# kevaday/alphazero-general

Measured on AMD Instinct MI355X. Metric: mcts_node_expansions_per_sec, higher is better.
Workload: dtype f32 tree / f16 net; 1 GPU; connect4 self-play, 2048 games/GPU x 100 sims/move, fp16 ResNet 128ch x 8, random-init, noise+temp on; games_per_gpu=2048, sims_per_move=100, hipgraph_rounds=True, stream_pipelines=1, fused_search_launch=True, mfma_tower=True, ranks=1

## Files before the change

alphazero_general_amd/csrc/azg_engine.hip:

```cpp
#include <hip/hip_runtime.h>
#include <hip/hip_ext.h>
#include <cstdio>
#include <cstdlib>
#include <cstring>
#include <map>
#include <mutex>
#include <string>
#include <vector>
#include "azg_kernels.h"
#include "azg_rules.h"
#include "azg_conv.h"
#include "azg_tiles.h"

using namespace azg;

static thread_local std::string g_err;
static int fail(int code, const std::string &msg) { g_err = msg; return code; }
#define HIPCHK(x) do { hipError_t _e = (x); if (_e != hipSuccess) return fail(AZG_E_HIP, std::string(#x) + ": " + hipGetErrorString(_e)); } while (0)

struct EvPair { hipEvent_t a, b; bool ext; };

static thread_local EvPair *g_kev = nullptr;
#define AZG_LAUNCH(kernel, grid, block, lds, stream, ...) do { \
    if (g_kev) { hipExtLaunchKernelGGL(kernel, grid, block, lds, stream, g_kev->a, g_kev->b, 0, __VA_ARGS__); g_kev = nullptr; } \
// ... 56 lines not shown
    e->allocs.push_back(q);
    *p = (T *)q;
    return AZG_OK;
}
#define DALLOC(ptr, count) do { int _r = dalloc(e, &(ptr), (size_t)(count)); if (_r != AZG_OK) return _r; } while (0)

#define AZG_GAME_CASE(G_, ...) case G_::ID: { using G = G_; __VA_ARGS__; } break;
#define GAME_SWITCH(e, ...) \
    switch ((e)->cfg.game) { AZG_GAMES(AZG_GAME_CASE, __VA_ARGS__) default: return fail(AZG_E_UNSUPPORTED, "game has no device rules"); }
#define AZG_SPARSE_CASE(G_, ...) case G_::ID: if constexpr (G_::SPARSE_HEADS) { using G = G_; __VA_ARGS__; } \
    else return fail(AZG_E_UNSUPPORTED, std::string("no sparse heads for ") + G_::NAME + " (use the dense heads)"); break;
#define SPARSE_GAME_SWITCH(e, ...) \
    switch ((e)->cfg.game) { AZG_GAMES(AZG_SPARSE_CASE, __VA_ARGS__) default: return fail(AZG_E_UNSUPPORTED, "game has no device rules"); }
#define OBS_SWITCH(obs_dtype, obs, CALL) \
    if ((obs_dtype) == 0) { using OBS = float; constexpr bool NHWC8 = false; OBS *const o = (OBS *)(obs); CALL; } \
    else if ((obs_dtype) == 1) { using OBS = _Float16; constexpr bool NHWC8 = false; OBS *const o = (OBS *)(obs); CALL; } \
    else { using OBS = _Float16; constexpr bool NHWC8 = true; OBS *const o = (OBS *)(obs); CALL; }

static void prof_begin(azg_engine *e, hipStream_t s, int fam, EvPair &p) {
    if (!e->profile) return;
    if (!e->pool.empty()) { p = e->pool.back(); e->pool.pop_back(); }
    else { (void)hipEventCreate(&p.a); (void)hipEventCreate(&p.b); }
    p.ext = fam != 2;
    if (p.ext) g_kev = &p; else (void)hipEventRecord(p.a, s);
}
static void prof_end(azg_engine *e, hipStream_t s, int fam, EvPair &p) {
    if (!e->profile) return;
    if (!p.ext) (void)hipEventRecord(p.b, s);
    g_kev = nullptr;
    e->ev[fam].push_back(p);
    e->launches[fam]++;
}
static void prof_drain(azg_engine *e) {
    for (int f = 0; f < 3; f++) {
        for (auto &p : e->ev[f]) {
            (void)hipEventSynchronize(p.b);
            float t = 0; (void)hipEventElapsedTime(&t, p.a, p.b);
            e->ms[f] += t;
            e->pool.push_back(p);
        }
        e->ev[f].clear();
    }
}

extern "C" int azg_engine_create(const azg_config *cfg, azg_engine **out) {
    if (!cfg || !out) return fail(AZG_E_INVALID_ARG, "null argument");
    if (cfg->abi_version != AZG_ABI_VERSION) return fail(AZG_E_INVALID_ARG, "ABI version mismatch");
    if (cfg->game < 0 || cfg->game >= k_num_games) return fail(AZG_E_UNSUPPORTED, "game has no device rules");
    if (cfg->num_slots <= 0) return fail(AZG_E_INVALID_ARG, "num_slots must be > 0");
    int ndev = 0;
    if (hipGetDeviceCount(&ndev) != hipSuccess || ndev == 0)
        return fail(AZG_E_HIP, "no HIP device: libazg_hip has no CPU fallback");
    HIPCHK(hipSetDevice(cfg->device));
    azg_engine *e = new azg_engine();
    e->cfg = *cfg; e->gi = k_info[cfg->game];
    const azg_game_info &gi = e->gi;
    View &v = e->v;
    memset(&v, 0, sizeof(v));
    v.B = cfg->num_slots; v.arena = cfg->arena ? 1 : 0; v.T = v.arena ? gi.num_players : 1;
    const int sims = cfg->sims_per_move > 0 ? cfg->sims_per_move : 100;
    const long long per_move = (long long)sims * gi.max_children;
    const long long cap = cfg->nodes_per_tree > 0 ? cfg->nodes_per_tree : (long long)(gi.max_turns < 16 ? gi.max_turns : 16) * per_move + 64;
    if (cap >= (1 << 28)) { delete e; return fail(AZG_E_INVALID_ARG, "nodes_per_tree must be < 2^28"); }
    v.cap = (int)cap;
    v.compact_reserve = (int)(per_move < cap / 2 ? per_move : cap / 2);
    v.maxd = gi.max_turns + 2; v.max_hist = gi.max_turns + 1;
    v.ex_cap = cfg->example_capacity; v.res_cap = cfg->result_capacity > 0 ? cfg->result_capacity : 4 * v.B + 1024;
    v.add_noise = (cfg->add_root_noise && !v.arena) ? 1 : 0; v.add_temp = (cfg->add_root_temp && !v.arena) ? 1 : 0;
    v.symmetric = cfg->symmetric_samples; v.reset_thr = cfg->mcts_reset_threshold; v.games_cap = cfg->games_per_iteration;
    v.cpuct = cfg->cpuct; v.fpu_reduction = cfg->fpu_reduction; v.noise_frac = cfg->root_noise_frac;
    v.root_temp = cfg->root_policy_temp; v.arena_temp = cfg->arena_temp;
    v.seed = cfg->tape_seed; v.slot_base = cfg->slot_base;
    const size_t trees = (size_t)v.B * v.T;
    const int A = gi.action_size, NV = gi.num_players + 1, O = gi.obs_c * gi.obs_h * gi.obs_w;
    DALLOC(v.nodes, trees * 2 * (size_t)v.cap);
    DALLOC(v.hdr, trees);
    DALLOC(v.path, trees * (size_t)v.maxd);
    DALLOC(v.states, v.B); DALLOC(v.leaf_states, v.B);
    DALLOC(v.tape_ctr, v.B); DALLOC(v.next_reset, v.B); DALLOC(v.hist_len, v.B);
    const bool hist = !v.arena && v.ex_cap > 0;
    DALLOC(v.hist_state, hist ? (size_t)v.B * v.max_hist : 1);
    DALLOC(v.hist_pi, hist ? (size_t)v.B * v.max_hist * A : 1);
    if (!hist) v.max_hist = 0;
    DALLOC(v.last_action, v.B); DALLOC(v.fin_flag, v.B); DALLOC(v.fin_ridx, v.B); DALLOC(v.fin_counted, v.B); DALLOC(v.fin_soff, v.B);
    DALLOC(v.slot_sims, v.B); DALLOC(v.slot_exp, v.B);
    DALLOC(v.gcount, 8);
    DALLOC(v.ex_obs, (size_t)v.ex_cap * O); DALLOC(v.ex_pi, (size_t)v.ex_cap * A); DALLOC(v.ex_z, (size_t)v.ex_cap * NV);
    DALLOC(v.res_ws, (size_t)v.res_cap * NV); DALLOC(v.res_turns, v.res_cap); DALLOC(v.res_slot, v.res_cap);
    std::vector<float> tt;
    if (cfg->temp_table && cfg->temp_table_len > 0) tt.assign(cfg->temp_table, cfg->temp_table + cfg->temp_table_len);
    else tt.assign(1, cfg->start_temp);
    float *d_tt; DALLOC(d_tt, tt.size());
    HIPCHK(hipMemcpy(d_tt, tt.data(), tt.size() * sizeof(float), hipMemcpyHostToDevice));
    v.temp_table = d_tt; v.temp_len = (int)tt.size();
    DALLOC(e->d_p2i, 8); DALLOC(e->d_ok, 4);
#ifdef AZG_TREE_TIMING
    DALLOC(v.dbg, (size_t)v.B * 16);
#endif
    *out = e;
    int r = azg_engine_reset(e, nullptr);
    if (r != AZG_OK) { azg_engine_destroy(e); *out = nullptr; return r; }
    HIPCHK(hipDeviceSynchronize());
    return AZG_OK;
}

extern "C" int azg_engine_destroy(azg_engine *e) {
    if (!e) return AZG_OK;
    (void)hipDeviceSynchronize();
    prof_drain(e);
    for (auto &p : e->pool) { (void)hipEventDestroy(p.a); (void)hipEventDestroy(p.b); }
    for (void *p : e->allocs) (void)hipFree(p);
    if (e->d_perm) (void)hipFree(e->d_perm);
    if (e->d_utape) (void)hipFree(e->d_utape);
    if (e->d_noff) (void)hipFree(e->d_noff);
    if (e->d_npool) (void)hipFree(e->d_npool);
    delete e;
    return AZG_OK;
}

extern "C" int azg_engine_reset(azg_engine *e, void *stream) {
    if (!e) return fail(AZG_E_INVALID_ARG, "null engine");
    hipStream_t s = (hipStream_t)stream;
    GAME_SWITCH(e, hipLaunchKernelGGL((k_reset<G>), dim3(e->v.B), dim3(64), 0, s, e->v, 0, e->v.B, 1));
    HIPCHK(hipMemsetAsync(e->v.tape_ctr, 0, sizeof(uint64_t) * e->v.B, s));
    HIPCHK(hipMemsetAsync(e->v.gcount, 0, sizeof(int32_t) * 8, s));
    HIPCHK(hipMemsetAsync(e->v.slot_sims, 0, sizeof(int64_t) * e->v.B, s));
    HIPCHK(hipMemsetAsync(e->v.slot_exp, 0, sizeof(int64_t) * e->v.B, s));
    HIPCHK(hipGetLastError());
    return AZG_OK;
}

static int check_range(azg_engine *e, int first, int count) {
    if (!e) return fail(AZG_E_INVALID_ARG, "null engine");
    if (first < 0 || count < 0 || first + count > e->v.B) return fail(AZG_E_INVALID_ARG, "slot range out of bounds");
    return AZG_OK;
}

extern "C" int azg_set_states(azg_engine *e, void *stream, int first, int count, const azg_state *host, int reset_trees) {
    int r = check_range(e, first, count); if (r) return r;
    hipStream_t s = (hipStream_t)stream;
    HIPCHK(hipMemcpyAsync(e->v.states + first, host, sizeof(azg_state) * count, hipMemcpyHostToDevice, s));
    if (reset_trees) { GAME_SWITCH(e, hipLaunchKernelGGL((k_reset<G>), dim3(count), dim3(64), 0, s, e->v, first, count, 0)); }
    HIPCHK(hipStreamSynchronize(s));
    return AZG_OK;
}
extern "C" int azg_get_states(azg_engine *e, void *stream, int first, int count, azg_state *host) {
    int r = check_range(e, first, count); if (r) return r;
    hipStream_t s = (hipStream_t)stream;
    HIPCHK(hipMemcpyAsync(host, e->v.states + first, sizeof(azg_state) * count, hipMemcpyDeviceToHost, s));
    HIPCHK(hipStreamSynchronize(s));
    return AZG_OK;
}
extern "C" int azg_get_leaf_states(azg_engine *e, void *stream, int first, int count, azg_state *host) {
    int r = check_range(e, first, count); if (r) return r;
    hipStream_t s = (hipStream_t)stream;
    HIPCHK(hipMemcpyAsync(host, e->v.leaf_states + first, sizeof(azg_state) * count, hipMemcpyDeviceToHost, s));
    HIPCHK(hipStreamSynchronize(s));
    return AZG_OK;
}
extern "C" int azg_set_tape_counters(azg_engine *e, void *stream, int first, int count, const uint64_t *host) {
    int r = check_range(e, first, count); if (r) return r;
    hipStream_t s = (hipStream_t)stream;
    HIPCHK(hipMemcpyAsync(e->v.tape_ctr + first, host, sizeof(uint64_t) * count, hipMemcpyHostToDevice, s));
    HIPCHK(hipStreamSynchronize(s));
    return AZG_OK;
}
extern "C" int azg_get_tape_counters(azg_engine *e, void *stream, int first, int count, uint64_t *host) {
// ... 54 lines not shown
    GAME_SWITCH(e, {
        RawValueRow<G> vrow;
        for (int j = 0; j < G::P + 1; j++) vrow.v[j] = value_host[j];
        hipLaunchKernelGGL((k_search_raw<G>), dim3(e->v.B), dim3(64), 0, s, e->v, policy_fill, vrow, sims);
    });
    HIPCHK(hipGetLastError());
    return AZG_OK;
}

extern "C" int azg_backup_select(azg_engine *e, void *stream, const float *policy, const float *value, const int32_t *row_of_slot, int flags,
                                 void *obs, int obs_dtype) {
    if (!e || !policy || !value) return fail(AZG_E_INVALID_ARG, "null argument");
    if (obs_dtype < 0 || obs_dtype > 2) return fail(AZG_E_INVALID_ARG, "obs_dtype must be 0 (f32), 1 (f16) or 2 (f16 NHWC8)");
    hipStream_t s = (hipStream_t)stream;
    View v = e->v;
    if (flags >= 0) { v.add_noise = (flags & AZG_FLAG_NOISE) ? 1 : 0; v.add_temp = (flags & AZG_FLAG_TEMP) ? 1 : 0; }
    EvPair p; prof_begin(e, s, 1, p);
    const int A = e->gi.action_size;
    OBS_SWITCH(obs_dtype, obs, GAME_SWITCH(e, AZG_LAUNCH((k_backup_select2<G, OBS, NHWC8, IN_PROBS>), dim3(v.B), dim3(128), 0, s, v, policy, value, A, o, row_of_slot, 1, HeadRows{})));
    prof_end(e, s, 1, p);
    HIPCHK(hipGetLastError());
    return AZG_OK;
}

extern "C" int azg_backup_select_logits(azg_engine *e, void *stream, const float *logits, int logits_stride, const int32_t *row_of_slot,
                                        int flags, void *obs, int obs_dtype, int do_select) {
    if (!e || !logits) return fail(AZG_E_INVALID_ARG, "null argument");
    if (obs_dtype < 0 || obs_dtype > 2) return fail(AZG_E_INVALID_ARG, "obs_dtype must be 0 (f32), 1 (f16) or 2 (f16 NHWC8)");
    if (logits_stride < e->gi.action_size + e->gi.num_players + 1 || e->gi.action_size > 1024)
        return fail(AZG_E_INVALID_ARG, "logits_stride must hold A + P + 1 logits (A <= 1024)");
    hipStream_t s = (hipStream_t)stream;
    View v = e->v;
    if (flags >= 0) { v.add_noise = (flags & AZG_FLAG_NOISE) ? 1 : 0; v.add_temp = (flags & AZG_FLAG_TEMP) ? 1 : 0; }
    EvPair p; prof_begin(e, s, 1, p);
    const float *nov = nullptr;
    OBS_SWITCH(obs_dtype, obs, GAME_SWITCH(e, AZG_LAUNCH((k_backup_select2<G, OBS, NHWC8, IN_LOGITS>), dim3(v.B), dim3(128), 0, s, v, logits, nov, logits_stride, o, row_of_slot, do_select, HeadRows{})));
    prof_end(e, s, 1, p);
    HIPCHK(hipGetLastError());
    return AZG_OK;
}

extern "C" int azg_backup_select_features(azg_engine *e, void *stream, const void *feat, int feat_k, const void *head_rows, const float *head_b,
                                          const int32_t *row_of_slot, int flags, void *obs, int obs_dtype, int do_select) {
    if (!e || !feat || !head_rows || !head_b) return fail(AZG_E_INVALID_ARG, "null argument");
    if (obs_dtype < 0 || obs_dtype > 2) return fail(AZG_E_INVALID_ARG, "obs_dtype must be 0 (f32), 1 (f16) or 2 (f16 NHWC8)");
    if (e->gi.action_size > 1024) return fail(AZG_E_INVALID_ARG, "A <= 1024");
    hipStream_t s = (hipStream_t)stream;
    View v = e->v;
    if (flags >= 0) { v.add_noise = (flags & AZG_FLAG_NOISE) ? 1 : 0; v.add_temp = (flags & AZG_FLAG_TEMP) ? 1 : 0; }
    const HeadRows hd{(const _Float16 *)head_rows, head_b, feat_k};
    int want = 0;
    SPARSE_GAME_SWITCH(e, want = head_fk<G>());
    if (feat_k != want) return fail(AZG_E_INVALID_ARG, "feat_k must be cells x 16 rounded up to a multiple of 32 for this game");
    EvPair p; prof_begin(e, s, 1, p);
    const float *nov = nullptr, *f = (const float *)feat;
    OBS_SWITCH(obs_dtype, obs, SPARSE_GAME_SWITCH(e, AZG_LAUNCH((k_backup_select2<G, OBS, NHWC8, IN_FEATURES>), dim3(v.B), dim3(128), 0, s, v, f, nov, 0, o, row_of_slot, do_select, hd)));
    prof_end(e, s, 1, p);
    HIPCHK(hipGetLastError());
    return AZG_OK;
}

extern "C" int azg_leaf_heads_sparse_f16(azg_engine *e, void *stream, const void *feat, int feat_k, const void *head_rows, const float *head_b,
                                         const int32_t *row_of_slot, float *logits, int logits_stride) {
    if (!e || !feat || !head_rows || !head_b || !logits) return fail(AZG_E_INVALID_ARG, "null argument");
    if (logits_stride < e->gi.action_size + e->gi.num_players + 1 || e->gi.action_size > 1024)
        return fail(AZG_E_INVALID_ARG, "logits_stride must hold A + P + 1 logits (A <= 1024)");
    int want = 0;
    SPARSE_GAME_SWITCH(e, want = head_fk<G>());
    if (feat_k != want) return fail(AZG_E_INVALID_ARG, "feat_k must be cells x 16 rounded up to a multiple of 32 for this game");
    const HeadRows hd{(const _Float16 *)head_rows, head_b, feat_k};
    SPARSE_GAME_SWITCH(e, hipLaunchKernelGGL((k_leaf_heads_sparse<G>), dim3(e->v.B), dim3(64), 0, (hipStream_t)stream, e->v, (const _Float16 *)feat, hd,
                                      row_of_slot, logits, logits_stride));
    HIPCHK(hipGetLastError());
    return AZG_OK;
}

extern "C" int azg_advance(azg_engine *e, void *stream, int record_history) {
    if (!e) return fail(AZG_E_INVALID_ARG, "null engine");
    hipStream_t s = (hipStream_t)stream;
    EvPair p; prof_begin(e, s, 2, p);
    GAME_SWITCH(e, {
        hipLaunchKernelGGL((k_play<G>), dim3(e->v.B), dim3(64), 0, s, e->v, record_history);
        hipLaunchKernelGGL((k_finalize<G>), dim3(1), dim3(64), 0, s, e->v, (const int32_t *)nullptr);
        hipLaunchKernelGGL((k_emit_samples<G>), dim3(e->v.B, G::NSYM), dim3(64), 0, s, e->v);
        hipLaunchKernelGGL((k_emit<G>), dim3(e->v.B), dim3(64), 0, s, e->v);
        hipLaunchKernelGGL((k_compact<G>), dim3(e->v.B * e->v.T), dim3(64), 0, s, e->v, 0, 0);
    });
    prof_end(e, s, 2, p);
    HIPCHK(hipGetLastError());
    return AZG_OK;
}

extern "C" int azg_advance_begin(azg_engine *e, void *stream, int record_history, int32_t *fin_host) {
    if (!e || !fin_host) return fail(AZG_E_INVALID_ARG, "null argument");
    hipStream_t s = (hipStream_t)stream;
    GAME_SWITCH(e, hipLaunchKernelGGL((k_play<G>), dim3(e->v.B), dim3(64), 0, s, e->v, record_history));
    HIPCHK(hipGetLastError());
    HIPCHK(hipMemcpyAsync(fin_host, e->v.fin_flag, sizeof(int32_t) * e->v.B, hipMemcpyDeviceToHost, s));
    HIPCHK(hipStreamSynchronize(s));
    return AZG_OK;
}

extern "C" int azg_advance_commit(azg_engine *e, void *stream, const int32_t *counted_host) {
    if (!e || !counted_host) return fail(AZG_E_INVALID_ARG, "null argument");
    hipStream_t s = (hipStream_t)stream;
    HIPCHK(hipMemcpyAsync(e->v.fin_counted, counted_host, sizeof(int32_t) * e->v.B, hipMemcpyHostToDevice, s));
    GAME_SWITCH(e, {
        hipLaunchKernelGGL((k_finalize<G>), dim3(1), dim3(64), 0, s, e->v, (const int32_t *)e->v.fin_counted);
        hipLaunchKernelGGL((k_emit_samples<G>), dim3(e->v.B, G::NSYM), dim3(64), 0, s, e->v);
        hipLaunchKernelGGL((k_emit<G>), dim3(e->v.B), dim3(64), 0, s, e->v);
        hipLaunchKernelGGL((k_compact<G>), dim3(e->v.B * e->v.T), dim3(64), 0, s, e->v, 0, 0);
    });
    HIPCHK(hipGetLastError());
    return AZG_OK;
}

extern "C" int azg_root_counts(azg_engine *e, void *stream, int32_t *counts) {
    if (!e || !counts) return fail(AZG_E_INVALID_ARG, "null argument");
    hipStream_t s = (hipStream_t)stream;
    GAME_SWITCH(e, hipLaunchKernelGGL((k_root_stats<G>), dim3(e->v.B), dim3(64), 0, s, e->v, 0, 1.0f, 0, counts, (float *)nullptr, (float *)nullptr));
    HIPCHK(hipGetLastError());
    return AZG_OK;
}
extern "C" int azg_root_probs(azg_engine *e, void *stream, float temp, float *probs) {
    if (!e || !probs) return fail(AZG_E_INVALID_ARG, "null argument");
    hipStream_t s = (hipStream_t)stream;
    GAME_SWITCH(e, hipLaunchKernelGGL((k_root_stats<G>), dim3(e->v.B), dim3(64), 0, s, e->v, 1, temp, 0, (int32_t *)nullptr, probs, (float *)nullptr));
    HIPCHK(hipGetLastError());
    return AZG_OK;
}
extern "C" int azg_root_value(azg_engine *e, void *stream, int average, float *values) {
    if (!e || !values) return fail(AZG_E_INVALID_ARG, "null argument");
    hipStream_t s = (hipStream_t)stream;
    GAME_SWITCH(e, hipLaunchKernelGGL((k_root_stats<G>), dim3(e->v.B), dim3(64), 0, s, e->v, 2, 1.0f, average, (int32_t *)nullptr, (float *)nullptr, values));
    HIPCHK(hipGetLastError());
    return AZG_OK;
}

extern "C" int azg_update_root(azg_engine *e, void *stream, int slot, int action) {
    int r = check_range(e, slot, 1); if (r) return r;
    hipStream_t s = (hipStream_t)stream;
    GAME_SWITCH(e, hipLaunchKernelGGL((k_update_root<G>), dim3(1), dim3(64), 0, s, e->v, slot, action, e->d_ok));
    GAME_SWITCH(e, hipLaunchKernelGGL((k_compact<G>), dim3(e->v.T), dim3(64), 0, s, e->v, 0, slot * e->v.T));
    int32_t ok = 0;
    HIPCHK(hipMemcpyAsync(&ok, e->d_ok, sizeof(ok), hipMemcpyDeviceToHost, s));
    HIPCHK(hipStreamSynchronize(s));
    if (!ok) return fail(AZG_E_INVALID_ACTION, "Invalid action encountered while updating root: " + std::to_string(action));
    return AZG_OK;
}

extern "C" int azg_compact(azg_engine *e, void *stream, int slot, int force) {
    if (!e) return fail(AZG_E_INVALID_ARG, "null engine");
    if (slot >= e->v.B) return fail(AZG_E_INVALID_ARG, "slot out of range");
    hipStream_t s = (hipStream_t)stream;
    const int first = slot < 0 ? 0 : slot * e->v.T, count = slot < 0 ? e->v.B * e->v.T : e->v.T;
    GAME_SWITCH(e, hipLaunchKernelGGL((k_compact<G>), dim3(count), dim3(64), 0, s, e->v, force ? 1 : 0, first));
    HIPCHK(hipGetLastError());
    return AZG_OK;
}

extern "C" int azg_engine_info(azg_engine *e, int32_t *out8) {
    if (!e || !out8) return fail(AZG_E_INVALID_ARG, "null argument");
    out8[0] = e->v.cap; out8[1] = e->v.compact_reserve; out8[2] = e->v.T; out8[3] = e->v.maxd; out8[4] = e->v.B;
    out8[5] = e->v.ex_cap; out8[6] = e->v.res_cap; out8[7] = e->cfg.sims_per_move > 0 ? e->cfg.sims_per_move : 100;
    return AZG_OK;
}

extern "C" int azg_set_random_tape(azg_engine *e, void *stream, const int16_t *ranks_host, const double *u_host, const int32_t *noise_off_host,
                                   const float *noise_pool_host, int noise_len, int len) {
    (void)stream;
    if (!e || len < 0 || noise_len < 0) return fail(AZG_E_INVALID_ARG, "null engine or negative length");
    if ((u_host || noise_off_host) && !ranks_host) return fail(AZG_E_INVALID_ARG, "choice / noise tapes come with a shuffle tape (one counter indexes all three)");
    if ((noise_off_host != nullptr) != (noise_pool_host != nullptr)) return fail(AZG_E_INVALID_ARG, "noise offsets and noise pool come together");
    const size_t n = (size_t)e->v.B * (size_t)(len > 0 ? len : 0);
    if (ranks_host) for (size_t i = 0; i < n; i++)
        if (ranks_host[i] < 0 || ranks_host[i] >= e->gi.max_children) return fail(AZG_E_INVALID_ARG, "shuffle tape: a rank is outside [0, max_children)");
    if (u_host) for (size_t i = 0; i < n; i++)
        if (!(u_host[i] >= 0.0 && u_host[i] < 1.0)) return fail(AZG_E_INVALID_ARG, "choice tape: a uniform is outside [0, 1)");
    if (noise_off_host) for (size_t i = 0; i < n; i++)
        if (noise_off_host[i] < -1 || noise_off_host[i] >= noise_len) return fail(AZG_E_INVALID_ARG, "noise tape: an offset is outside the pool");
    HIPCHK(hipDeviceSynchronize());
    if (e->d_perm) { (void)hipFree(e->d_perm); e->d_perm = nullptr; }
    if (e->d_utape) { (void)hipFree(e->d_utape); e->d_utape = nullptr; }
    if (e->d_noff) { (void)hipFree(e->d_noff); e->d_noff = nullptr; }
    if (e->d_npool) { (void)hipFree(e->d_npool); e->d_npool = nullptr; }
    e->v.perm_tape = nullptr; e->v.perm_len = 0; e->v.u_tape = nullptr; e->v.noise_off = nullptr; e->v.noise_pool = nullptr; e->v.noise_len = 0;
    if (!ranks_host || len == 0) return AZG_OK;
    HIPCHK(hipMalloc((void **)&e->d_perm, n * sizeof(int16_t)));
    HIPCHK(hipMemcpy(e->d_perm, ranks_host, n * sizeof(int16_t), hipMemcpyHostToDevice));
    if (u_host) {
        HIPCHK(hipMalloc((void **)&e->d_utape, n * sizeof(double)));
        HIPCHK(hipMemcpy(e->d_utape, u_host, n * sizeof(double), hipMemcpyHostToDevice));
    }
    if (noise_off_host) {
// ... 970 lines not shown
```

alphazero_general_amd/csrc/azg_kernels.h:

```cpp
#pragma once
#include "azg_games.h"

namespace azg {

struct NodeR {
    int n; float q, p, v; int fc; int a, nchild, player, e;
};
AZG_DEV void unpack(const uint4 &lo, const uint4 &hi, NodeR &r) {
    r.n = (int)lo.x; r.q = __uint_as_float(lo.y); r.p = __uint_as_float(lo.z); r.v = __uint_as_float(lo.w);
    r.fc = (int)hi.x; r.a = hi.y & 0xFFFF; r.nchild = hi.y >> 16; r.player = hi.z & 0xFF; r.e = (hi.z >> 8) & 0xFF;
}
AZG_DEV uint4 pack_hi(int fc, int a, int nchild, int player, int e) {
    return make_uint4((unsigned)fc, (unsigned)(a & 0xFFFF) | ((unsigned)nchild << 16), (unsigned)player | ((unsigned)e << 8), 0u);
}
AZG_DEV void load_node(const Node *p, uint4 &lo, uint4 &hi) {
    const uint4 *q = reinterpret_cast<const uint4 *>(p);
    lo = q[0]; hi = q[1];
}
AZG_DEV void raise_error(const View &ev, int code) { atomicCAS(&ev.gcount[GC_ERROR], 0, code); }
#ifdef AZG_DEBUG_BOUNDS
AZG_DEV bool bounds_fail(const View &ev, int site) { raise_error(ev, AZG_E_INTERNAL); atomicCAS(&ev.gcount[GC_BOUNDS_SITE], 0, site); return false; }
#define AZG_BOUNDS_OK(ev, site, cond) ((cond) ? true : bounds_fail(ev, site))
#else
#define AZG_BOUNDS_OK(ev, site, cond) true
// ... 788 lines not shown
    else s = np_sum_static<A>(cnt, scr, lane);
    const double ex = 1.0 / (double)temp;
    for (int a = lane; a < A; a += 64) pr[a] = np_pow_f32(cnt[a] / s, ex);
    wave_sync();
    float s2;
    if constexpr (A < 8) { s2 = 0.f; for (int a = 0; a < A; a++) s2 += pr[a]; }
    else s2 = np_sum_static<A>(pr, scr, lane);
    for (int a = lane; a < A; a += 64) pr[a] = pr[a] / s2;
    wave_sync();
}

template <class G>
__global__ __launch_bounds__(64) void k_root_stats(View ev, int what, float temp, int average, int32_t *counts, float *probs, float *values) {
    constexpr int A = G::A;
    __shared__ float cnt[A < 8 ? 8 : A], pr[A < 8 ? 8 : A], scr[64];
    const int slot = blockIdx.x, lane = threadIdx.x;
    const int mover0 = __builtin_amdgcn_readfirstlane(ev.states[slot].player);
    const int tree = ev.arena ? slot * ev.T + mover0 : slot;
    HdrR hr; load_hdr(ev.hdr + tree, hr);
    const Node *nodes = tree_nodes(ev, tree, hr.base);
    const int fc = hr.root.fc, k = hr.root.nchild;
    if (k > 0 && !AZG_BLOCK_OK(ev, 11, fc, k, hr.alloc)) return;
    if (what == 0) {
        for (int a = lane; a < A; a += 64) counts[(size_t)slot * A + a] = 0;
        wave_sync();
        for (int i = lane; i < k; i += 64) counts[(size_t)slot * A + nodes[fc + i].a] = nodes[fc + i].n;
    } else if (what == 1) {
        root_probs<G>(ev, nodes, fc, k, temp, cnt, pr, scr, lane);
        for (int a = lane; a < A; a += 64) probs[(size_t)slot * A + a] = pr[a];
    } else if (lane == 0) {
        float value = 0.f;
        if (average) {
            double s = 0.0;
            for (int i = 0; i < k; i++) if (nodes[fc + i].n > 0) s += (double)nodes[fc + i].q;
            value = (float)(s / (double)k);
        } else {
            for (int i = 0; i < k; i++) if (nodes[fc + i].q > value && nodes[fc + i].n > 0) value = nodes[fc + i].q;
        }
        values[slot] = value;
    }
}

template <class G>
AZG_DEV bool update_root(const View &ev, int slot, int tree, const typename G::S &st, int action, int *act_lds, int lane) {
    constexpr int NCH = (G::MAXK + 63) / 64;
    TreeHdr *h = ev.hdr + tree;
    HdrR hr; load_hdr(h, hr);
    Node *nodes = tree_nodes(ev, tree, hr.base);
    int fc = hr.root.fc, k = hr.root.nchild;
    if (k == 0) {
        int my_a[NCH];
        k = G::valid_list(st, lane, act_lds, my_a);
        uint64_t ctr = ev.tape_ctr[slot];
        int alloc = hr.alloc;
        fc = add_children_any<G>(ev, slot, nodes, alloc, k, my_a, ctr, lane, NoRanks{});
        if (fc < 0) return false;
        if (lane == 0) { ev.tape_ctr[slot] = ctr; h->alloc = alloc; }
        wave_sync();
    }
    int found = -1;
    if (!AZG_BLOCK_OK(ev, 7, fc, k, __builtin_amdgcn_readfirstlane(h->alloc))) return false;
    for (int i0 = 0; i0 < k; i0 += 64) {
        int i = i0 + lane;
        uint64_t bal = __ballot(i < k && (int)nodes[fc + i].a == action);
        if (bal) { found = i0 + __ffsll((unsigned long long)bal) - 1; break; }
    }
    if (found < 0) return false;
    uint4 lo, hi; load_node(nodes + fc + found, lo, hi);
    if (lane == 0) { uint4 *q = reinterpret_cast<uint4 *>(h); q[0] = lo; q[1] = hi; }
    return true;
}

template <class G>
__global__ __launch_bounds__(64) void k_update_root(View ev, int slot, int action, int32_t *ok) {
    __shared__ int act_lds[((G::MAXK + 63) / 64) * 64];
    const int lane = threadIdx.x;
    typename G::S st = G::load(&ev.states[slot], lane);
    bool good = true;
    for (int t = 0; t < ev.T; t++) good = update_root<G>(ev, slot, slot * ev.T + t, st, action, act_lds, lane) && good;
    if (lane == 0) *ok = good ? 1 : 0;
}

template <class G>
__global__ __launch_bounds__(64) void k_compact(View ev, int force, int first_tree) {
    if (__builtin_amdgcn_readfirstlane(ev.gcount[GC_ERROR]) != 0) return;
    const int tree = first_tree + blockIdx.x, lane = threadIdx.x;
    TreeHdr *h = ev.hdr + tree;
    HdrR hr; load_hdr(h, hr);
    if (!force && hr.alloc + ev.compact_reserve <= ev.cap) return;
    const Node *from = tree_nodes(ev, tree, hr.base);
    const int nbase = hr.base ? 0 : ev.cap;
    Node *to = tree_nodes(ev, tree, nbase);
    int nalloc = 0;
    if (hr.root.fc >= 0 && hr.root.nchild > 0) {
        const int k = hr.root.nchild;
        if (!AZG_BLOCK_OK(ev, 8, hr.root.fc, k, hr.alloc)) return;
        for (int i = lane; i < k; i += 64) { uint4 lo, hi; load_node(from + hr.root.fc + i, lo, hi); uint4 *q = reinterpret_cast<uint4 *>(to + i); q[0] = lo; q[1] = hi; }
        nalloc = k;
    }
    wave_sync();
    for (int scan = 0; scan < nalloc;) {
        const int end = min(scan + 64, nalloc), i = scan + lane;
        scan = end;
        int ofc = -1, kk = 0;
        if (i < end) { const uint4 hi = reinterpret_cast<const uint4 *>(to + i)[1]; ofc = (int)hi.x; kk = ofc >= 0 ? (int)(hi.y >> 16) : 0; }
        const int off = wave_excl_scan(kk, lane), total = wave_sum_i(kk);
        const int nfc = nalloc + off;
        if (kk > 0) reinterpret_cast<int32_t *>(to + i)[4] = nfc;
        uint64_t todo = __ballot(kk > 0);
        while (todo) {
            const int b = __ffsll((unsigned long long)todo) - 1; todo &= todo - 1;
            const int sfc = rl(ofc, b), sk = rl(kk, b), dfc = rl(nfc, b);
            if (!AZG_BLOCK_OK(ev, 9, sfc, sk, hr.alloc) || !AZG_BOUNDS_OK(ev, 10, dfc >= 0 && dfc + sk <= ev.cap)) continue;
            for (int j = lane; j < sk; j += 64) { uint4 lo, hi; load_node(from + sfc + j, lo, hi); uint4 *q = reinterpret_cast<uint4 *>(to + dfc + j); q[0] = lo; q[1] = hi; }
        }
        nalloc += total;
        wave_sync();
    }
    if (lane == 0) {
        if (hr.root.fc >= 0 && hr.root.nchild > 0) h->root.first_child = 0;
        h->base = nbase; h->alloc = nalloc;
        atomicMax(&ev.gcount[GC_MAXLIVE], nalloc);
        h->leaf = LEAF_IS_ROOT; h->leaf_fc = -1; h->depth = 0;
    }
}

template <class G>
__global__ __launch_bounds__(64) void k_play(View ev, int record_history) {
    if (__builtin_amdgcn_readfirstlane(ev.gcount[GC_ERROR]) != 0) return;
    constexpr int A = G::A;
    __shared__ float cnt[A < 8 ? 8 : A], pr[A < 8 ? 8 : A], scr[64];
    __shared__ int act_lds[((G::MAXK + 63) / 64) * 64];
    const int slot = blockIdx.x, lane = threadIdx.x;
    typename G::S st = G::load(&ev.states[slot], lane);
    if (G::win_bits(st) != 0) {
        if (lane == 0) ev.fin_flag[slot] = 0;
        return;
    }
    const int tree = ev.arena ? slot * ev.T + st.player : slot;
    HdrR hr; load_hdr(ev.hdr + tree, hr);
    const Node *nodes = tree_nodes(ev, tree, hr.base);
    const int fc = hr.root.fc, k = hr.root.nchild;
    if (k > 0 && !AZG_BLOCK_OK(ev, 11, fc, k, hr.alloc)) return;
    float temp;
    if (ev.arena) temp = ev.arena_temp;
    else { int t = st.turns < ev.temp_len ? st.turns : ev.temp_len - 1; temp = ev.temp_table[t]; }
    root_probs<G>(ev, nodes, fc, k, temp, cnt, pr, scr, lane);
    {
        bool nan = false;
        for (int a = lane; a < A; a += 64) nan |= pr[a] != pr[a];
        if (__ballot(nan)) { if (lane == 0) { raise_error(ev, AZG_E_FLOATING_POINT); ev.fin_flag[slot] = 0; } return; }
    }
    uint64_t ctr = ev.tape_ctr[slot];
    double u;
    if (ev.u_tape) {
        if (ctr >= (uint64_t)ev.perm_len) { if (lane == 0) { raise_error(ev, AZG_E_INVALID_ARG); ev.fin_flag[slot] = 0; } return; }
        u = ev.u_tape[(size_t)slot * ev.perm_len + ctr];
    } else u = u53(tape_u64(ev.seed, ev.slot_base + (uint64_t)slot, ctr));
    double total = 0.0;
    for (int a = 0; a < A; a++) { float x = pr[a]; if (x != 0.f) total += (double)x; }
    double acc = 0.0; int action = 0; bool le = true;
    for (int a = 0; a < A; a++) {
        float x = pr[a];
        if (x != 0.f) { acc += (double)x; le = (acc / total) <= u; }
        if (le) action = a + 1;
    }
    if (action >= A) action = A - 1;
    wave_sync();
    if (lane == 0) { ev.tape_ctr[slot] = ctr + 1; ev.last_action[slot] = action; }
    if (record_history && !ev.arena && ev.max_hist > 0) {
        const int hl = __builtin_amdgcn_readfirstlane(ev.hist_len[slot]);
        if (hl < ev.max_hist) {
            if (temp != 1.0f) root_probs<G>(ev, nodes, fc, k, 1.0f, cnt, pr, scr, lane);
            float *hp = ev.hist_pi + ((size_t)slot * ev.max_hist + hl) * A;
            for (int a = lane; a < A; a += 64) hp[a] = pr[a];
            G::store(st, &ev.hist_state[(size_t)slot * ev.max_hist + hl], lane);
            if (lane == 0) ev.hist_len[slot] = hl + 1;
        } else if (lane == 0) raise_error(ev, AZG_E_EXAMPLES_FULL);
    }
    wave_sync();
    bool ok = true;
    if (ev.arena) { for (int t = 0; t < ev.T; t++) ok = update_root<G>(ev, slot, slot * ev.T + t, st, action, act_lds, lane) && ok; }
    else ok = update_root<G>(ev, slot, tree, st, action, act_lds, lane);
    if (!ok && lane == 0) raise_error(ev, AZG_E_INVALID_ACTION);
    G::play(st, action);
    if (ev.reset_thr) {
        const int nr = __builtin_amdgcn_readfirstlane(ev.next_reset[slot]);
        if (st.turns >= nr) {
            for (int t = 0; t < ev.T; t++) init_tree(ev, slot * ev.T + t, lane);
            if (lane == 0) ev.next_reset[slot] = st.turns + ev.reset_thr;
        }
    }
    const int ws = G::win_bits(st);
    G::store(st, &ev.states[slot], lane);
    if (lane == 0) ev.fin_flag[slot] = ws;
}

template <class G>
__global__ __launch_bounds__(64) void k_finalize(View ev, const int32_t *counted_in) {
    if (__builtin_amdgcn_readfirstlane(ev.gcount[GC_ERROR]) != 0) return;
    const int lane = threadIdx.x;
    const int nsym = ev.symmetric ? G::NSYM : 1;
    int gp = ev.gcount[GC_GAMES], nr = ev.gcount[GC_RESULTS], ne = ev.gcount[GC_EXAMPLES];
    for (int s0 = 0; s0 < ev.B; s0 += 64) {
        const int s = s0 + lane;
        const int fin = s < ev.B ? (ev.fin_flag[s] != 0) : 0;
        const int rank = wave_excl_scan(fin, lane);
        const int counted = counted_in ? (fin && counted_in[s] != 0) : (fin && (gp + rank < ev.games_cap));
        const int ns = (counted && !ev.arena) ? ev.hist_len[s] * nsym : 0;
        const int soff = wave_excl_scan(ns, lane);
        if (fin) { ev.fin_ridx[s] = nr + rank; ev.fin_counted[s] = counted; ev.fin_soff[s] = ne + soff; }
        const int nfin = wave_sum_i(fin), ncnt = wave_sum_i(counted), nsum = wave_sum_i(ns);
        gp += ncnt; nr += nfin; ne += nsum;
    }
    if (lane == 0) {
        if (nr > ev.res_cap || (ev.ex_cap > 0 && ne > ev.ex_cap)) raise_error(ev, AZG_E_EXAMPLES_FULL);
        ev.gcount[GC_GAMES] = gp; ev.gcount[GC_RESULTS] = nr; ev.gcount[GC_EXAMPLES] = ne;
    }
}

template <class G>
__global__ __launch_bounds__(64) void k_emit_samples(View ev) {
    if (__builtin_amdgcn_readfirstlane(ev.gcount[GC_ERROR]) != 0) return;
    constexpr int A = G::A, NV = G::P + 1;
    const int slot = blockIdx.x, kk = blockIdx.y, lane = threadIdx.x;
    const int ws = __builtin_amdgcn_readfirstlane(ev.fin_flag[slot]);
    if (ws == 0 || !ev.fin_counted[slot] || ev.arena || ev.ex_cap <= 0) return;
    const int nsym = ev.symmetric ? G::NSYM : 1;
    if (kk >= nsym) return;
    const int hl = ev.hist_len[slot], soff = ev.fin_soff[slot];
    for (int hI = 0; hI < hl; hI++) {
        const int si = soff + hI * nsym + kk;
        if (si >= ev.ex_cap) continue;
        typename G::S hs = G::load(&ev.hist_state[(size_t)slot * ev.max_hist + hI], lane);
        const float *hp = ev.hist_pi + ((size_t)slot * ev.max_hist + hI) * A;
        const int k = ev.symmetric ? kk : G::SYM_RAW;
        typename G::S ss = G::symmetry(hs, k);
        G::template write_obs<float>(ss, ev.ex_obs + (size_t)si * G::OBS, lane);
        for (int a = lane; a < A; a += 64) ev.ex_pi[(size_t)si * A + G::sym_action(a, k)] = hp[a];
        if (lane < NV) ev.ex_z[(size_t)si * NV + lane] = (float)((ws >> lane) & 1);
    }
}

template <class G>
__global__ __launch_bounds__(64) void k_emit(View ev) {
    if (__builtin_amdgcn_readfirstlane(ev.gcount[GC_ERROR]) != 0) return;
    constexpr int A = G::A, NV = G::P + 1;
    const int slot = blockIdx.x, lane = threadIdx.x;
    const int ws = __builtin_amdgcn_readfirstlane(ev.fin_flag[slot]);
    if (ws == 0) return;
    const int ridx = ev.fin_ridx[slot], counted = ev.fin_counted[slot];
    if (ridx < ev.res_cap && lane == 0) {
        for (int j = 0; j < NV; j++) ev.res_ws[(size_t)ridx * NV + j] = (uint8_t)((ws >> j) & 1);
        ev.res_turns[ridx] = ev.states[slot].turns; ev.res_slot[ridx] = slot;
    }
    if (!counted) return;
    typename G::S st; G::init(st);
    G::store(st, &ev.states[slot], lane);
    if (lane == 0) ev.hist_len[slot] = 0;
    for (int t = 0; t < ev.T; t++) init_tree(ev, slot * ev.T + t, lane);
}

template <class G>
__global__ __launch_bounds__(64) void k_reset(View ev, int first, int count, int reset_state) {
    const int slot = first + blockIdx.x, lane = threadIdx.x;
    if (slot >= first + count) return;
    if (reset_state) { typename G::S st; G::init(st); G::store(st, &ev.states[slot], lane); }
    if (lane == 0) { ev.hist_len[slot] = 0; ev.next_reset[slot] = 0; ev.fin_flag[slot] = 0; }
    for (int t = 0; t < ev.T; t++) init_tree(ev, slot * ev.T + t, lane);
}

__global__ __launch_bounds__(256) void k_max_nodes(View ev) {
    int m = 0;
    for (int t = threadIdx.x; t < ev.B * ev.T; t += 256) m = max(m, ev.hdr[t].alloc);
    atomicMax(&ev.gcount[GC_MAXNODES], m);
}

__global__ __launch_bounds__(64) void k_reset_max_depth(View ev) {
    const int t = blockIdx.x * 64 + threadIdx.x;
    if (t < ev.B * ev.T) ev.hdr[t].max_depth = 0;
}

struct SeatMap { int32_t v[8]; };

__global__ __launch_bounds__(64) void k_arena_rows(View ev, SeatMap seat, const uint32_t *seat_of_slot, int32_t *row_of_slot,
                                                   int32_t *rows_per_model) {
    const int lane = threadIdx.x;
    const int32_t *p2i = seat.v;
    int base = 0;
    for (int mi = 0; mi < ev.T; mi++) {
        int cntm = 0;
        for (int s0 = 0; s0 < ev.B; s0 += 64) {
            const int s = s0 + lane;
            int is = 0;
            if (s < ev.B) {
                const int mover = ev.states[s].player;
                is = (seat_of_slot ? (int)((seat_of_slot[s] >> (4 * mover)) & 15u) : p2i[mover]) == mi;
            }
            const int r = wave_excl_scan(is, lane);
            if (is) row_of_slot[s] = base + cntm + r;
            cntm += wave_sum_i(is);
        }
        if (lane == 0) rows_per_model[mi] = cntm;
        base += cntm;
    }
}

}
```

Measured before the change: 7.919 million expansions/s.

## Fuse emit_samples, emit and compact into one per-tree kernel with finished-game list

Merges the sample emission, result emission and tree compaction kernels into a single kernel launched per tree. k_finalize now builds a compact list of finished games with sample offsets, so sample writing is spread over blocks instead of launching B x NSYM mostly idle blocks. The serial action draw in k_play is replaced with a wave-parallel ballot-based draw. This cuts launches and idle blocks in the advance step, at the cost of more complex indexing (a binary search over the list) and changed finalize and draw code that must match the previous semantics.

```diff
diff --git a/alphazero_general_amd/csrc/azg_engine.hip b/alphazero_general_amd/csrc/azg_engine.hip
--- a/alphazero_general_amd/csrc/azg_engine.hip
+++ b/alphazero_general_amd/csrc/azg_engine.hip
@@ -162,7 +162,8 @@
     DALLOC(v.hist_state, hist ? (size_t)v.B * v.max_hist : 1);
     DALLOC(v.hist_pi, hist ? (size_t)v.B * v.max_hist * A : 1);
     if (!hist) v.max_hist = 0;
-    DALLOC(v.last_action, v.B); DALLOC(v.fin_flag, v.B); DALLOC(v.fin_ridx, v.B); DALLOC(v.fin_counted, v.B); DALLOC(v.fin_soff, v.B);
+    DALLOC(v.last_action, v.B); DALLOC(v.fin_flag, v.B); DALLOC(v.fin_ridx, v.B); DALLOC(v.fin_counted, v.B);
+    DALLOC(v.fin_soff, fin_list_offset(v.B) + 4 * ((size_t)v.B + 1));
     DALLOC(v.slot_sims, v.B); DALLOC(v.slot_exp, v.B);
     DALLOC(v.gcount, 8);
     DALLOC(v.ex_obs, (size_t)v.ex_cap * O); DALLOC(v.ex_pi, (size_t)v.ex_cap * A); DALLOC(v.ex_z, (size_t)v.ex_cap * NV);
@@ -383,9 +384,7 @@
     GAME_SWITCH(e, {
         hipLaunchKernelGGL((k_play<G>), dim3(e->v.B), dim3(64), 0, s, e->v, record_history);
         hipLaunchKernelGGL((k_finalize<G>), dim3(1), dim3(64), 0, s, e->v, (const int32_t *)nullptr);
-        hipLaunchKernelGGL((k_emit_samples<G>), dim3(e->v.B, G::NSYM), dim3(64), 0, s, e->v);
-        hipLaunchKernelGGL((k_emit<G>), dim3(e->v.B), dim3(64), 0, s, e->v);
-        hipLaunchKernelGGL((k_compact<G>), dim3(e->v.B * e->v.T), dim3(64), 0, s, e->v, 0, 0);
+        hipLaunchKernelGGL((k_emit<G>), dim3(e->v.B * e->v.T), dim3(64), 0, s, e->v);
     });
     prof_end(e, s, 2, p);
     HIPCHK(hipGetLastError());
@@ -408,9 +407,7 @@
     HIPCHK(hipMemcpyAsync(e->v.fin_counted, counted_host, sizeof(int32_t) * e->v.B, hipMemcpyHostToDevice, s));
     GAME_SWITCH(e, {
         hipLaunchKernelGGL((k_finalize<G>), dim3(1), dim3(64), 0, s, e->v, (const int32_t *)e->v.fin_counted);
-        hipLaunchKernelGGL((k_emit_samples<G>), dim3(e->v.B, G::NSYM), dim3(64), 0, s, e->v);
-        hipLaunchKernelGGL((k_emit<G>), dim3(e->v.B), dim3(64), 0, s, e->v);
-        hipLaunchKernelGGL((k_compact<G>), dim3(e->v.B * e->v.T), dim3(64), 0, s, e->v, 0, 0);
+        hipLaunchKernelGGL((k_emit<G>), dim3(e->v.B * e->v.T), dim3(64), 0, s, e->v);
     });
     HIPCHK(hipGetLastError());
     return AZG_OK;
diff --git a/alphazero_general_amd/csrc/azg_kernels.h b/alphazero_general_amd/csrc/azg_kernels.h
--- a/alphazero_general_amd/csrc/azg_kernels.h
+++ b/alphazero_general_amd/csrc/azg_kernels.h
@@ -894,9 +894,7 @@
 }
 
 template <class G>
-__global__ __launch_bounds__(64) void k_compact(View ev, int force, int first_tree) {
-    if (__builtin_amdgcn_readfirstlane(ev.gcount[GC_ERROR]) != 0) return;
-    const int tree = first_tree + blockIdx.x, lane = threadIdx.x;
+AZG_DEV void compact_tree(const View &ev, int tree, int force, int lane) {
     TreeHdr *h = ev.hdr + tree;
     HdrR hr; load_hdr(h, hr);
     if (!force && hr.alloc + ev.compact_reserve <= ev.cap) return;
@@ -936,14 +934,111 @@
         h->leaf = LEAF_IS_ROOT; h->leaf_fc = -1; h->depth = 0;
     }
 }
-
-template <class G>
-__global__ __launch_bounds__(64) void k_play(View ev, int record_history) {
+template <class G>
+__global__ __launch_bounds__(64) void k_compact(View ev, int force, int first_tree) {
     if (__builtin_amdgcn_readfirstlane(ev.gcount[GC_ERROR]) != 0) return;
+    compact_tree<G>(ev, first_tree + blockIdx.x, force, threadIdx.x);
+}
+
+template <int A>
+AZG_HD int draw_action_serial(const float *pr, double u) {
+    double total = 0.0;
+    for (int a = 0; a < A; a++) { float x = pr[a]; if (x != 0.f) total += (double)x; }
+    double acc = 0.0; int action = 0; bool le = true;
+    for (int a = 0; a < A; a++) {
+        float x = pr[a];
+        if (x != 0.f) { acc += (double)x; le = (acc / total) <= u; }
+        if (le) action = a + 1;
+    }
+    return action >= A ? A - 1 : action;
+}
+template <int A>
+AZG_DEV int draw_action(const float *pr, double u, int lane) {
+    double total = 0.0;
+    for (int a0 = 0; a0 < A; a0 += 64) {
+        const float x = a0 + lane < A ? pr[a0 + lane] : 0.f;
+        uint64_t nz = __ballot(x != 0.f);
+        while (nz) { const int b = __ffsll((unsigned long long)nz) - 1; nz &= nz - 1; total += (double)rl(x, b); }
+    }
+    double acc = 0.0, my_acc = 0.0;
+    int my_a = 0, j = 0;
+    for (int a0 = 0; a0 < A; a0 += 64) {
+        const float x = a0 + lane < A ? pr[a0 + lane] : 0.f;
+        uint64_t nz = __ballot(x != 0.f);
+        while (nz) {
+            const int b = __ffsll((unsigned long long)nz) - 1; nz &= nz - 1;
+            acc += (double)rl(x, b);
+            if (lane == (j & 63)) { my_acc = acc; my_a = a0 + b; }
+            j++;
+            if ((j & 63) == 0) {
+                const uint64_t gt = __ballot(!((my_acc / total) <= u));
+                if (gt) return rl(my_a, __ffsll((unsigned long long)gt) - 1);
+            }
+        }
+    }
+    const uint64_t gt = __ballot(lane < (j & 63) && !((my_acc / total) <= u));
+    if (gt) return rl(my_a, __ffsll((unsigned long long)gt) - 1);
+    return A - 1;
+}
+
+AZG_HD size_t fin_list_offset(int B) { return ((size_t)B + 3) & ~(size_t)3; }
+AZG_DEV int4 *fin_list(const View &ev) { return reinterpret_cast<int4 *>(ev.fin_soff + fin_list_offset(ev.B)); }
+
+template <class G>
+AZG_DEV void finalize_scan(const View &ev, const int32_t *counted_in, int lane) {
+    constexpr int PER = 16;
+    const int nsym = ev.symmetric ? G::NSYM : 1;
+    const bool samples = !ev.arena;
+    int gp = ev.gcount[GC_GAMES], nr = ev.gcount[GC_RESULTS], ne = ev.gcount[GC_EXAMPLES], nl = 0;
+    const int ne0 = ne;
+    int4 *list = fin_list(ev);
+    for (int c0 = 0; c0 < ev.B; c0 += 64 * PER) {
+        const int s0 = c0 + lane * PER;
+        int fl[PER], hl[PER], cin[PER];
+#pragma unroll
+        for (int i = 0; i < PER; i++) {
+            const bool in = s0 + i < ev.B;
+            fl[i] = in ? ev.fin_flag[s0 + i] : 0;
+            hl[i] = in ? ev.hist_len[s0 + i] : 0;
+            cin[i] = (in && counted_in) ? counted_in[s0 + i] : 0;
+        }
+        int nf = 0;
+#pragma unroll
+        for (int i = 0; i < PER; i++) nf += fl[i] != 0;
+        const int rank0 = wave_excl_scan(nf, lane), nfin = wave_sum_i(nf);
+        unsigned cbits = 0;
+        int ns = 0, nc = 0, nm = 0;
+#pragma unroll
+        for (int i = 0, r = rank0; i < PER; i++) {
+            const bool fin = fl[i] != 0;
+            const bool counted = fin && (counted_in ? cin[i] != 0 : gp + r < ev.games_cap);
+            r += fin;
+            if (counted) { cbits |= 1u << i; nc++; }
+            const int n = (counted && samples) ? hl[i] * nsym : 0;
+            ns += n; nm += n > 0;
+        }
+        const int soff0 = wave_excl_scan(ns, lane), m0 = wave_excl_scan(nm, lane);
+#pragma unroll
+        for (int i = 0, r = rank0, so = soff0, m = m0; i < PER; i++) {
+            if (fl[i] == 0) continue;
+            const int s = s0 + i, counted = (cbits >> i) & 1;
+            const int n = (counted && samples) ? hl[i] * nsym : 0;
+            ev.fin_ridx[s] = nr + r; ev.fin_counted[s] = counted; ev.fin_soff[s] = ne + so;
+            if (n > 0) { list[1 + nl + m] = make_int4(s, hl[i], ne + so, fl[i]); m++; }
+            r++; so += n;
+        }
+        gp += wave_sum_i(nc); nr += nfin; ne += wave_sum_i(ns); nl += wave_sum_i(nm);
+    }
+    if (lane == 0) {
+        if (nr > ev.res_cap || (ev.ex_cap > 0 && ne > ev.ex_cap)) raise_error(ev, AZG_E_EXAMPLES_FULL);
+        ev.gcount[GC_GAMES] = gp; ev.gcount[GC_RESULTS] = nr; ev.gcount[GC_EXAMPLES] = ne;
+        list[0] = make_int4(nl, ev.ex_cap > 0 ? ne - ne0 : 0, ne0, 0);
+    }
+}
+
+template <class G>
+AZG_DEV void play_slot(const View &ev, int slot, int record_history, float *cnt, float *pr, float *scr, int *act_lds, int lane) {
     constexpr int A = G::A;
-    __shared__ float cnt[A < 8 ? 8 : A], pr[A < 8 ? 8 : A], scr[64];
-    __shared__ int act_lds[((G::MAXK + 63) / 64) * 64];
-    const int slot = blockIdx.x, lane = threadIdx.x;
     typename G::S st = G::load(&ev.states[slot], lane);
     if (G::win_bits(st) != 0) {
         if (lane == 0) ev.fin_flag[slot] = 0;
@@ -969,15 +1064,10 @@
         if (ctr >= (uint64_t)ev.perm_len) { if (lane == 0) { raise_error(ev, AZG_E_INVALID_ARG); ev.fin_flag[slot] = 0; } return; }
         u = ev.u_tape[(size_t)slot * ev.perm_len + ctr];
     } else u = u53(tape_u64(ev.seed, ev.slot_base + (uint64_t)slot, ctr));
-    double total = 0.0;
-    for (int a = 0; a < A; a++) { float x = pr[a]; if (x != 0.f) total += (double)x; }
-    double acc = 0.0; int action = 0; bool le = true;
-    for (int a = 0; a < A; a++) {
-        float x = pr[a];
-        if (x != 0.f) { acc += (double)x; le = (acc / total) <= u; }
-        if (le) action = a + 1;
-    }
-    if (action >= A) action = A - 1;
+    const int action = draw_action<A>(pr, u, lane);
+#ifdef AZG_DEBUG_BOUNDS
+    if (!AZG_BOUNDS_OK(ev, 12, action == draw_action_serial<A>(pr, u))) return;
+#endif
     wave_sync();
     if (lane == 0) { ev.tape_ctr[slot] = ctr + 1; ev.last_action[slot] = action; }
     if (record_history && !ev.arena && ev.max_hist > 0) {
@@ -1009,68 +1099,75 @@
 }
 
 template <class G>
+__global__ __launch_bounds__(64) void k_play(View ev, int record_history) {
+    if (__builtin_amdgcn_readfirstlane(ev.gcount[GC_ERROR]) != 0) return;
+    constexpr int A = G::A;
+    __shared__ float cnt[A < 8 ? 8 : A], pr[A < 8 ? 8 : A], scr[64];
+    __shared__ int act_lds[((G::MAXK + 63) / 64) * 64];
+    play_slot<G>(ev, blockIdx.x, record_history, cnt, pr, scr, act_lds, threadIdx.x);
+}
+
+template <class G>
 __global__ __launch_bounds__(64) void k_finalize(View ev, const int32_t *counted_in) {
     if (__builtin_amdgcn_readfirstlane(ev.gcount[GC_ERROR]) != 0) return;
-    const int lane = threadIdx.x;
-    const int nsym = ev.symmetric ? G::NSYM : 1;
-    int gp = ev.gcount[GC_GAMES], nr = ev.gcount[GC_RESULTS], ne = ev.gcount[GC_EXAMPLES];
-    for (int s0 = 0; s0 < ev.B; s0 += 64) {
-        const int s = s0 + lane;
-        const int fin = s < ev.B ? (ev.fin_flag[s] != 0) : 0;
-        const int rank = wave_excl_scan(fin, lane);
-        const int counted = counted_in ? (fin && counted_in[s] != 0) : (fin && (gp + rank < ev.games_cap));
-        const int ns = (counted && !ev.arena) ? ev.hist_len[s] * nsym : 0;
-        const int soff = wave_excl_scan(ns, lane);
-        if (fin) { ev.fin_ridx[s] = nr + rank; ev.fin_counted[s] = counted; ev.fin_soff[s] = ne + soff; }
-        const int nfin = wave_sum_i(fin), ncnt = wave_sum_i(counted), nsum = wave_sum_i(ns);
-        gp += ncnt; nr += nfin; ne += nsum;
-    }
-    if (lane == 0) {
-        if (nr > ev.res_cap || (ev.ex_cap > 0 && ne > ev.ex_cap)) raise_error(ev, AZG_E_EXAMPLES_FULL);
-        ev.gcount[GC_GAMES] = gp; ev.gcount[GC_RESULTS] = nr; ev.gcount[GC_EXAMPLES] = ne;
-    }
-}
-
-template <class G>
-__global__ __launch_bounds__(64) void k_emit_samples(View ev) {
+    finalize_scan<G>(ev, counted_in, threadIdx.x);
+}
+
+template <class G>
+__global__ __launch_bounds__(64) void k_emit(View ev) {
     if (__builtin_amdgcn_readfirstlane(ev.gcount[GC_ERROR]) != 0) return;
     constexpr int A = G::A, NV = G::P + 1;
-    const int slot = blockIdx.x, kk = blockIdx.y, lane = threadIdx.x;
-    const int ws = __builtin_amdgcn_readfirstlane(ev.fin_flag[slot]);
-    if (ws == 0 || !ev.fin_counted[slot] || ev.arena || ev.ex_cap <= 0) return;
+    const int tree = blockIdx.x, lane = threadIdx.x;
+    const int slot = tree / ev.T, t0 = tree - slot * ev.T == 0;
+    const int4 *list = fin_list(ev);
+    const int4 rec = lane <= ev.B ? list[lane] : make_int4(0, 0, 0, 0);
+    const int ws = ev.fin_flag[slot], ridx = ev.fin_ridx[slot], counted = ev.fin_counted[slot];
+    const int nent = rl(rec.x, 0), first = rl(rec.z, 0);
+    const int items = (ev.arena || ev.ex_cap <= 0 || nent <= 0 || nent > ev.B) ? 0 : rl(rec.y, 0);
     const int nsym = ev.symmetric ? G::NSYM : 1;
-    if (kk >= nsym) return;
-    const int hl = ev.hist_len[slot], soff = ev.fin_soff[slot];
-    for (int hI = 0; hI < hl; hI++) {
-        const int si = soff + hI * nsym + kk;
+    for (int i = blockIdx.x; i < items; i += gridDim.x) {
+        const int si = first + i;
         if (si >= ev.ex_cap) continue;
-        typename G::S hs = G::load(&ev.hist_state[(size_t)slot * ev.max_hist + hI], lane);
-        const float *hp = ev.hist_pi + ((size_t)slot * ev.max_hist + hI) * A;
+        int e = __popcll(__ballot(lane >= 1 && lane <= nent && rec.z <= si));
+        int4 en;
+        if (e == 0) continue;
+        if (e < 63 || nent <= 63) en = make_int4(rl(rec.x, e), rl(rec.y, e), rl(rec.z, e), rl(rec.w, e));
+        else {
+            int hi = nent;
+            while (e < hi) {
+                const int mid = (e + hi + 1) >> 1;
+                if (__builtin_amdgcn_readfirstlane(list[mid].z) <= si) e = mid; else hi = mid - 1;
+            }
+            en = list[e];
+        }
+        const int es = __builtin_amdgcn_readfirstlane(en.x), hl = __builtin_amdgcn_readfirstlane(en.y);
+        const int j = si - __builtin_amdgcn_readfirstlane(en.z), ews = __builtin_amdgcn_readfirstlane(en.w);
+        const int hI = j / nsym, kk = j - hI * nsym;
+        if (j < 0 || hI >= hl || hl > ev.max_hist || es < 0 || es >= ev.B) continue;
+        typename G::S hs = G::load(&ev.hist_state[(size_t)es * ev.max_hist + hI], lane);
+        const float *hp = ev.hist_pi + ((size_t)es * ev.max_hist + hI) * A;
         const int k = ev.symmetric ? kk : G::SYM_RAW;
         typename G::S ss = G::symmetry(hs, k);
         G::template write_obs<float>(ss, ev.ex_obs + (size_t)si * G::OBS, lane);
         for (int a = lane; a < A; a += 64) ev.ex_pi[(size_t)si * A + G::sym_action(a, k)] = hp[a];
-        if (lane < NV) ev.ex_z[(size_t)si * NV + lane] = (float)((ws >> lane) & 1);
-    }
-}
-
-template <class G>
-__global__ __launch_bounds__(64) void k_emit(View ev) {
-    if (__builtin_amdgcn_readfirstlane(ev.gcount[GC_ERROR]) != 0) return;
-    constexpr int A = G::A, NV = G::P + 1;
-    const int slot = blockIdx.x, lane = threadIdx.x;
-    const int ws = __builtin_amdgcn_readfirstlane(ev.fin_flag[slot]);
-    if (ws == 0) return;
-    const int ridx = ev.fin_ridx[slot], counted = ev.fin_counted[slot];
-    if (ridx < ev.res_cap && lane == 0) {
-        for (int j = 0; j < NV; j++) ev.res_ws[(size_t)ridx * NV + j] = (uint8_t)((ws >> j) & 1);
-        ev.res_turns[ridx] = ev.states[slot].turns; ev.res_slot[ridx] = slot;
-    }
-    if (!counted) return;
-    typename G::S st; G::init(st);
-    G::store(st, &ev.states[slot], lane);
-    if (lane == 0) ev.hist_len[slot] = 0;
-    for (int t = 0; t < ev.T; t++) init_tree(ev, slot * ev.T + t, lane);
+        if (lane < NV) ev.ex_z[(size_t)si * NV + lane] = (float)((ews >> lane) & 1);
+    }
+    if (__builtin_amdgcn_readfirstlane(ws) != 0) {
+        if (t0 && ridx < ev.res_cap && lane == 0) {
+            for (int j = 0; j < NV; j++) ev.res_ws[(size_t)ridx * NV + j] = (uint8_t)((ws >> j) & 1);
+            ev.res_turns[ridx] = ev.states[slot].turns; ev.res_slot[ridx] = slot;
+        }
+        if (__builtin_amdgcn_readfirstlane(counted)) {
+            if (t0) {
+                typename G::S st; G::init(st);
+                G::store(st, &ev.states[slot], lane);
+                if (lane == 0) ev.hist_len[slot] = 0;
+            }
+            init_tree(ev, tree, lane);
+            wave_sync();
+        }
+    }
+    compact_tree<G>(ev, tree, 0, lane);
 }
 
 template <class G>
```

Measured after the change: 7.906 million expansions/s. No clear change (-0.2%).
